# 0411tony/Yue

Hardware: AMD Instinct MI355X
Metric: BPR triplet-updates/sec at k=128 (S-round semantics, user rows sequential; the reference's exact sequential semantics: secondary.exact) (higher is better)
Workload: dtype f32

## Files before the change

include/yue_hip.h:

```cpp
#ifndef YUE_HIP_H
#define YUE_HIP_H

#include <stdint.h>

#ifdef __cplusplus
extern "C" {
#endif

typedef struct yue_ctx yue_ctx;

#define YUE_OK              0
#define YUE_ERR_ARG        -1
#define YUE_ERR_HIP        -2
#define YUE_ERR_FEW_ITEMS  -3
#define YUE_ERR_COMM       -4
#define YUE_ERR_SATURATED  -5

#define YUE_MAX_ATTEMPTS   64
#define YUE_UNIQUE_ID_BYTES 128

const char *yue_last_error(void);
int yue_version(void);

int yue_ctx_create(int device, yue_ctx **out);
// ... 19 lines not shown

int yue_bpr_rounds(yue_ctx *ctx, const int32_t *u, const int32_t *i, const int32_t *j,
                   const int64_t *round_ptr, int64_t n_rounds,
                   double lr, double regU, double regI, double *nll_out);

int yue_bpr_epoch(yue_ctx *ctx, uint64_t seed, uint32_t epoch, int64_t round_events,
                  double lr, double regU, double regI,
                  double *nll_out, double *sumsqP_out, double *sumsqQ_out);

int yue_epoch_plan(int64_t m, int k, int64_t round_events, double events_total, int nranks,
                   int64_t *user_block, int64_t *blocks_per_group, int64_t *n_blocks);

int yue_default_round_events(yue_ctx *ctx, int64_t *out);

int yue_sample_negatives(yue_ctx *ctx, uint64_t seed, uint32_t epoch, int32_t *j_out);

int yue_sumsq(yue_ctx *ctx, double *sumsqP_out, double *sumsqQ_out);

int yue_scores(yue_ctx *ctx, int32_t user, float *out_n);

int yue_topn_scan(yue_ctx *ctx, const int32_t *users, int64_t nu, int N,
                  const int64_t *mask_indptr, const int32_t *mask_indices,
                  int32_t *out_ids, float *out_scores);

int yue_set_kernel_timing(yue_ctx *ctx, int stride);
int yue_get_kernel_timing(yue_ctx *ctx, double *total_ms, int64_t *launches_timed, int64_t *triplets_timed);
int yue_get_scan_stats(yue_ctx *ctx, double *kernel_ms, int64_t *events, int64_t *rescored, int *used_bf16);
int yue_get_scan_work(yue_ctx *ctx, int64_t *tiles_scored, int64_t *tiles_total);

int yue_set_option(yue_ctx *ctx, const char *name, int64_t value);
// ... 99 lines not shown
```

yue_amd/_shim.py:

```python
import ctypes as C
import os

import numpy as np

_HERE = os.path.dirname(os.path.abspath(__file__))
LIB_PATH = os.path.join(_HERE, 'csrc', 'libyue_hip.so')

OK, ERR_ARG, ERR_HIP, ERR_FEW_ITEMS, ERR_COMM, ERR_SATURATED = 0, -1, -2, -3, -4, -5
UNIQUE_ID_BYTES = 128

SYMBOLS = ['yue_last_error', 'yue_version', 'yue_ctx_create', 'yue_ctx_destroy', 'yue_sync',
           'yue_set_factors', 'yue_get_factors', 'yue_set_interactions', 'yue_bpr_replay',
           'yue_bpr_rounds', 'yue_bpr_epoch', 'yue_cune_steps', 'yue_adam_reset', 'yue_adam_get_moments', 'yue_adam_step', 'yue_sample_negatives', 'yue_sumsq', 'yue_scores',
           'yue_topn_scan', 'yue_set_kernel_timing', 'yue_get_kernel_timing', 'yue_get_scan_stats', 'yue_get_scan_work', 'yue_set_option', 'yue_get_option',
           'yue_comm_unique_id', 'yue_comm_init', 'yue_allreduce_f64', 'yue_get_comm_stats',
           'yue_default_round_events', 'yue_epoch_plan',
           'yue_fism_set_model', 'yue_fism_get_model', 'yue_fism_epoch', 'yue_fism_rounds', 'yue_fism_scores', 'yue_fism_topn_scan',
           'yue_wrmf_set_pairs', 'yue_wrmf_half_sweep',
           'yue_expo_set_pairs', 'yue_expo_set_mu', 'yue_expo_get_mu', 'yue_expo_half_sweep', 'yue_expo_update_mu', 'yue_expo_gram_rows',
           'yue_cof_cooccur', 'yue_cof_get_cooccur', 'yue_cof_set_sppmi', 'yue_cof_set_state', 'yue_cof_get_state', 'yue_cof_item_sweep',
           'yue_knn_set_pairs', 'yue_knn_neighbors', 'yue_knn_predict', 'yue_knn_topn',
           'yue_ipf_set_graph', 'yue_ipf_predict', 'yue_ipf_topn',
           'yue_cnet_set_pairs', 'yue_cnet_walks', 'yue_cnet_set_walks', 'yue_cnet_set_sentences', 'yue_cnet_embed', 'yue_cnet_set_embedding',
           'yue_cnet_friends',
           'yue_s2v_set_state', 'yue_s2v_get_state', 'yue_s2v_set_steps', 'yue_s2v_set_pairs', 'yue_s2v_epoch',
           'yue_lgcn_set_graph', 'yue_lgcn_propagate', 'yue_lgcn_grad', 'yue_lgcn_step',
           'yue_ngcf_set_graph', 'yue_ngcf_set_weights', 'yue_ngcf_get_weights', 'yue_ngcf_propagate', 'yue_ngcf_grad', 'yue_ngcf_step',
           'yue_cdae_set_data', 'yue_cdae_set_params', 'yue_cdae_get_params', 'yue_cdae_forward', 'yue_cdae_grad', 'yue_cdae_step',
# ... 338 lines not shown
    def default_round_events(self):
        out = C.c_int64()
        self._chk(self._lib.yue_default_round_events(self._ctx, C.byref(out)))
        return out.value

    def bpr_epoch(self, seed, epoch, round_events, lr, regU, regI):
        nll, sp, sq = C.c_double(), C.c_double(), C.c_double()
        self._chk(self._lib.yue_bpr_epoch(self._ctx, C.c_uint64(seed), C.c_uint32(epoch), C.c_int64(round_events), C.c_double(lr), C.c_double(regU),
                                          C.c_double(regI), C.byref(nll), C.byref(sp), C.byref(sq)))
        return nll.value, sp.value, sq.value

    def sample_negatives(self, seed, epoch):
        j = np.empty(max(self.E, 1), np.int32)
        self._chk(self._lib.yue_sample_negatives(self._ctx, C.c_uint64(seed), C.c_uint32(epoch), j.ctypes.data_as(C.POINTER(C.c_int32))))
        return j[:self.E]

    def sumsq(self):
        sp, sq = C.c_double(), C.c_double()
        self._chk(self._lib.yue_sumsq(self._ctx, C.byref(sp), C.byref(sq)))
        return sp.value, sq.value

    def scores(self, user):
        out = np.empty(self.n, np.float32)
        self._chk(self._lib.yue_scores(self._ctx, C.c_int32(user), out.ctypes.data_as(C.POINTER(C.c_float))))
        return out

    def topn_scan(self, users, N, mask_indptr=None, mask_indices=None):
        users, up = _i32(users)
        ids = np.empty((len(users), N), np.int32)
        sc = np.empty((len(users), N), np.float32)
# ... 366 lines not shown
```

yue_amd/csrc/bpr_device.hpp:

```cpp
#pragma once
#include <hip/hip_runtime.h>
#include <stdint.h>

namespace yue {

constexpr int kNllSlots = 1024;
constexpr int kMaxAttempts = 64;

struct TrainArgs {
    float *P, *Q, *dP, *dQ;
    float *stage;
#ifdef YUE_STAMPS
    unsigned long long *stamps;
#endif
    const int32_t *ev_u, *ev_i;
    int32_t *ev_j;
    const int64_t *indptr;
    const int32_t *indices;
    double *nll_slots;
    int64_t m, n;
    int k;
    float ru, ri;
    double lr;
    uint64_t seed;
// ... 7 lines not shown
    unsigned long long *cnt_cur;
    unsigned long long *cnt_next;
    uint32_t *cntp_cur;
    uint32_t *cntp_next;
    uint32_t *tab_cur, *tab_next;
    int staged;
    int apply_p;
};

__device__ __forceinline__ uint64_t mix64(uint64_t z) {
    z ^= z >> 30; z *= 0xBF58476D1CE4E5B9ull;
    z ^= z >> 27; z *= 0x94D049BB133111EBull;
    z ^= z >> 31; return z;
}

__device__ __forceinline__ int32_t ctr_draw(uint64_t seed, uint32_t epoch, uint64_t e, uint32_t a, int32_t lo, int32_t n_range) {
    uint64_t z = mix64(seed + 0x9E3779B97F4A7C15ull * (e + 1));
    z = mix64(z ^ (0xD1B54A32D192ED03ull * (uint64_t)(epoch + 1) + 0x8CB92BA72F3D8DD7ull * (uint64_t)a));
    return lo + (int32_t)(((z >> 32) * (uint64_t)(uint32_t)n_range) >> 32);
}

__device__ __forceinline__ bool csr_contains(const int64_t *indptr, const int32_t *indices, int64_t row, int32_t x) {
    int64_t lo = indptr[row], hi = indptr[row + 1];
    while (lo < hi) {
        int64_t mid = (lo + hi) >> 1;
        int32_t v = indices[mid];
        if (v < x) lo = mid + 1; else if (v > x) hi = mid; else return true;
    }
    return false;
}

__device__ __forceinline__ int32_t sample_negative(const TrainArgs &a, int32_t u, int64_t e) {
    for (uint32_t t = 0; t < (uint32_t)kMaxAttempts; ++t) {
        int32_t c = ctr_draw(a.seed, a.epoch, (uint64_t)e, t, a.neg_lo, a.neg_range);
// ... 111 lines not shown
```

yue_amd/csrc/bpr_host.hip:

```cpp
#include "host_common.hpp"

#include "train_kernels.hpp"
#include "round_kernels.hpp"

using yue_host::fail;
using yue_host::kr_of;
using yue_host::with_kr;
static_assert(yue::kNllSlots == yue_host::kNllSlotsHost && yue::kHeaderSlack == yue_host::kHeaderSlackHost &&
              yue::kMetaStageMax == (uint32_t)yue_host::kMetaStageMaxHost, "host_common.hpp mirrors these");

namespace {

yue::TrainArgs make_args(yue_ctx *c, double lr, double regU, double regI) {
    yue::TrainArgs a{};
    a.P = c->P.p; a.Q = c->Q.p; a.dP = c->dP.p; a.dQ = c->dQ.p;
    a.stage = c->Q.p ? c->Q.p + (size_t)c->n * c->k : nullptr;
    a.ev_u = c->ev_u.p; a.ev_i = c->ev_i.p; a.ev_j = c->ev_j.p;
    a.indptr = c->indptr.p; a.indices = c->indices.p;
    a.nll_slots = c->scal.p;
    a.m = c->m; a.n = c->n; a.k = c->k;
    a.lr = lr;
    a.ru = (float)(lr * regU);
    a.ri = (float)(lr * regI);
    a.neg_lo = 0; a.neg_range = (int32_t)c->n;
// ... 182 lines not shown
            }
        });
        if (!is_default) return fail(YUE_ERR_ARG, "item matrices of 2 GiB and more: only the default events-per-wave setting (round_tpw = 0)");
    } else if (!with_round_instance(kr_of(c->k), tpw, [&](auto kr, auto t) {
                   hipLaunchKernelGGL((yue::k_round_m<kr(), t()>), grid, block, 0, c->stream, a, ra, a.ev_u, a.ev_i, a.ev_j, mi, mj);
               }))
        return fail(YUE_ERR_ARG, "unsupported (k, TPW) combination");
    launch_round_fold(c, a, e0, e1, round_index);
    return YUE_OK;
}

int launch_round_u(yue_ctx *c, const yue::TrainArgs &a, int64_t u0, int64_t u1, int64_t e0, int64_t e1, int64_t round_index) {
    yue::RoundUArgs ra{};
    ra.u_begin = u0; ra.u_end = u1; ra.ev_ptr = c->d_ev_ptr.p; ra.e_begin = e0; ra.e_end = e1; ra.staged = c->staged ? 1 : 0; ra.margins = c->margins.p;
    ra.psq_slots = c->psq_in_rounds ? c->psq_slots.p : nullptr;
    const int64_t blocks = (u1 - u0 + 3) / 4;
    if (blocks == 0) return YUE_OK;
    const dim3 grid((unsigned)blocks), block(256);
    const uint32_t *mi = c->meta_i.p, *mj = c->meta_j.p;
    with_kr(c->k, [&](auto kr) {
        if (c->opt_round_fast) hipLaunchKernelGGL((yue::k_round_u<kr(), true>), grid, block, 0, c->stream, a, ra, a.ev_i, a.ev_j, mi, mj);
        else hipLaunchKernelGGL((yue::k_round_u<kr(), false>), grid, block, 0, c->stream, a, ra, a.ev_i, a.ev_j, mi, mj);
    });
    launch_round_fold(c, a, e0, e1, round_index);
    return YUE_OK;
}

template <typename F>
int run_rounds(yue_ctx *c, yue::TrainArgs a, const std::vector<int64_t> &bounds, int apply_p, F after_round, bool meta = false, const std::vector<int64_t> *user_blocks = nullptr) {
    const int64_t R = (int64_t)bounds.size() - 1;
// ... 54 lines not shown
                      : meta ? launch_round_m(c, a, e0, e1, r) : launch_round(c, a, e0, e1, n0, n1, (int)(pos & 1), apply_p))) return rc;
            ++pos;
        }
        if ((rc = after_round(r))) return rc;
    }
    if (timed) {
        HIPCHK(hipEventRecord(c->ev_pool[c->ev_used].second, c->stream));
        c->ev_triplets[c->ev_used] = bounds.back() - bounds.front();
        c->ev_launches[c->ev_used] = (int64_t)ne.size();
        c->ev_used++;
    }
    return YUE_OK;
}

void reset_round_state(yue_ctx *c) {
    (void)hipStreamSynchronize(c->stream);
    if (c->cnt0.p) (void)hipMemsetAsync(c->cnt0.p, 0, c->cnt0.n * sizeof(unsigned long long), c->stream);
    if (c->cnt1.p) (void)hipMemsetAsync(c->cnt1.p, 0, c->cnt1.n * sizeof(unsigned long long), c->stream);
    if (c->cntp0.p) (void)hipMemsetAsync(c->cntp0.p, 0, c->cntp0.n * sizeof(uint32_t), c->stream);
    if (c->cntp1.p) (void)hipMemsetAsync(c->cntp1.p, 0, c->cntp1.n * sizeof(uint32_t), c->stream);
    if (c->dP.p) (void)hipMemsetAsync(c->dP.p, 0, c->dP.n * sizeof(float), c->stream);
    if (c->dQ.p) (void)hipMemsetAsync(c->dQ.p, 0, c->dQ.n * sizeof(float), c->stream);
    (void)hipStreamSynchronize(c->stream);
}

}

namespace yue_host {
bool fold_path(const yue_ctx *c) { return meta_path_fits(c); }

// ... 190 lines not shown
    int rc = upload_triplets(c, u, i, j, T, true);
    if (rc) return rc;
    if ((rc = zero_scalars(c))) return rc;
    yue::MbArgs a{};
    a.U = c->P.p; a.V = c->Q.p; a.gU = c->dP.p; a.gV = c->dQ.p; a.k = c->k; a.u = c->xu.p; a.i = c->xi.p; a.j = c->xj.p; a.T = T;
    a.reg = (float)reg; a.loss_slots = c->scal.p;
    const dim3 grid((unsigned)(((T + 31) / 32 + 3) / 4));
    with_kr(c->k, [&](auto kr) { hipLaunchKernelGGL(yue::k_mb_grad<kr()>, grid, dim3(256), 0, c->stream, a); });
    if ((rc = yue_host::adam_apply(c, lr, step))) return rc;
    return read_scalars(c, loss_out, nullptr, nullptr);
}

int yue_sample_negatives(yue_ctx *c, uint64_t seed, uint32_t epoch, int32_t *j_out) {
    if (!c || !c->have_inter || !j_out) return fail(YUE_ERR_ARG, "yue_sample_negatives: no interactions uploaded");
    HIPCHK(hipSetDevice(c->device));
    yue::TrainArgs a = make_args(c, 0, 0, 0);
    a.seed = seed; a.epoch = epoch;
    if (c->E > 0) {
        hipLaunchKernelGGL(yue::k_sample, dim3((unsigned)((c->E + 255) / 256)), dim3(256), 0, c->stream, a, c->E);
        HIPCHK(hipGetLastError());
        HIPCHK(hipMemcpyAsync(j_out, c->ev_j.p, c->E * sizeof(int32_t), hipMemcpyDeviceToHost, c->stream));
    }
    HIPCHK(hipStreamSynchronize(c->stream));
    return YUE_OK;
}

int yue_sumsq(yue_ctx *c, double *sp, double *sq) {
    if (!c || !c->have_factors) return fail(YUE_ERR_ARG, "yue_sumsq: no factors uploaded");
    HIPCHK(hipSetDevice(c->device));
    int rc = sumsq_async(c);
    if (rc) return rc;
    double h[2];
    HIPCHK(hipMemcpyAsync(h, c->scal.p + yue::kNllSlots + 1, sizeof h, hipMemcpyDeviceToHost, c->stream));
    HIPCHK(hipStreamSynchronize(c->stream));
    if (sp) *sp = h[0];
    if (sq) *sq = h[1];
    return YUE_OK;
}

int yue_bpr_epoch(yue_ctx *c, uint64_t seed, uint32_t epoch, int64_t round_events, double lr, double regU, double regI,
                  double *nll_out, double *sumsqP_out, double *sumsqQ_out) {
    if (!c || !c->have_factors || !c->have_inter) return fail(YUE_ERR_ARG, "yue_bpr_epoch: upload factors and interactions first");
    if (round_events < 0) return fail(YUE_ERR_ARG, "yue_bpr_epoch: round_events must be positive (or 0 for the device's default)");
    HIPCHK(hipSetDevice(c->device));
    yue::TrainArgs a = make_args(c, lr, regU, regI);
    a.seed = seed + 0x632BE59BD9B4E019ull * (uint64_t)c->rank;
    a.epoch = epoch;
    int rc = zero_scalars(c);
    if (rc) return rc;
    const int64_t E = c->E;
    if (E > 0) hipLaunchKernelGGL(yue::k_sample, dim3((unsigned)((E + 255) / 256)), dim3(256), 0, c->stream, a, E);
    if (c->opt_epoch_exact) {
        if (yue_host::on_communicator(c) && c->nranks > 1) return fail(YUE_ERR_ARG, "yue_bpr_epoch: option epoch_exact runs on one GPU (the sequential order spans all item shards)");
        if ((rc = yue_host::chain_epoch(c, lr, regU, regI))) return rc;
        if ((rc = sumsq_async(c))) return rc;
        return read_scalars(c, nll_out, sumsqP_out, sumsqQ_out);
    }
    std::vector<int64_t> bounds;
    double tot[2] = {(double)E, (double)c->n};
    if (yue_host::on_communicator(c)) {
        if ((rc = yue_allreduce_f64(c, tot, 2))) return rc;
        if ((rc = zero_scalars(c))) return rc;
    }
    const double etot = tot[0];
    if (round_events == 0 && (rc = default_round_events(c, tot[1] / c->nranks, &round_events))) return rc;
    int64_t ub = 1, group = 1;
// ... 26 lines not shown
        const int64_t first = g_first * c->k, count = (g_last - g_first) * c->k;
        const dim3 grid((unsigned)std::min<int64_t>(4096, (count + 255) / 256));
        if (!yue_host::on_communicator(c)) {
            hipLaunchKernelGGL(yue::k_apply_range, grid, dim3(256), 0, c->stream, c->P.p, c->dP.p, first, count);
            return YUE_OK;
        }
        HIPCHK(hipEventRecord(c->ev_rounds, c->stream));
        HIPCHK(hipStreamWaitEvent(c->comm_stream, c->ev_rounds, 0));
        c->comm_collectives += 1;
        c->comm_bytes += (double)count * sizeof(float);
        if (const int rcr = yue_host::reduce_user_block(c, first, count, c->comm_stream)) return rcr;
        hipLaunchKernelGGL(yue::k_apply_range, grid, dim3(256), 0, c->comm_stream, c->P.p, c->dP.p, first, count);
        return YUE_OK;
    };
    c->comm_collectives = 0; c->comm_bytes = 0.0; c->comm_wait_ms = 0.0;
    if ((rc = run_rounds(c, a, bounds, 0, after, meta_path_fits(c), seq_user ? &ublock : nullptr))) { reset_round_state(c); return rc; }
    if (c->last_round_user_seq && E > 0)
        hipLaunchKernelGGL(yue::k_loss_margins, dim3(2048), dim3(256), 0, c->stream, c->margins.p, c->ev_j.p, E, c->scal.p);
    const bool psq_done = c->psq_in_rounds && c->last_round_user_seq;
    c->psq_in_rounds = false;
    if (yue_host::on_communicator(c)) {
        HIPCHK(hipEventRecord(c->ev_t_rounds, c->stream));
        HIPCHK(hipEventRecord(c->ev_t_comm, c->comm_stream));
    }
    HIPCHK(hipEventRecord(c->ev_comm, c->comm_stream));
    HIPCHK(hipStreamWaitEvent(c->stream, c->ev_comm, 0));
    c->comm_compute_waits = 1;
    HIPCHK(hipGetLastError());
    if ((rc = sumsq_async(c, psq_done ? c->psq_slots.p : nullptr))) return rc;
    if ((rc = read_scalars(c, nll_out, sumsqP_out, sumsqQ_out))) return rc;
    if (yue_host::on_communicator(c)) {
        float ms = 0.f;
        HIPCHK(hipEventSynchronize(c->ev_t_comm));
        HIPCHK(hipEventElapsedTime(&ms, c->ev_t_rounds, c->ev_t_comm));
        c->comm_wait_ms = ms > 0.f ? ms : 0.0;
    }
    return YUE_OK;
}

int yue_epoch_plan(int64_t m, int k, int64_t round_events, double events_total, int nranks,
                   int64_t *user_block, int64_t *blocks_per_group, int64_t *n_blocks) {
    if (m <= 0 || k <= 0 || round_events <= 0 || nranks < 1 || !(events_total >= 0.0)) return fail(YUE_ERR_ARG, "yue_epoch_plan: bad argument");
    const double per_user = events_total / (double)nranks / (double)m;
    const int64_t ub = std::max<int64_t>(1, (int64_t)std::floor((double)round_events / std::max(per_user, 1e-9) + 0.5));
    if (user_block) *user_block = ub;
    if (blocks_per_group) *blocks_per_group = std::max<int64_t>(1, (8ll << 20) / std::max<int64_t>(1, ub * k * 4));
    if (n_blocks) *n_blocks = (m + ub - 1) / ub;
    return YUE_OK;
}

int yue_default_round_events(yue_ctx *c, int64_t *out) {
// ... 50 lines not shown
```

yue_amd/csrc/core_host.hip:

```cpp
#include "host_common.hpp"

namespace yue_host {
thread_local std::string g_err;
int fail(int code, const std::string &msg) { g_err = msg; return code; }
}
using yue_host::fail;
void yue_comm_release(yue_ctx *c);

extern "C" {

const char *yue_last_error(void) { return yue_host::g_err.c_str(); }
int yue_version(void) { return 1; }

int yue_ctx_create(int device, yue_ctx **out) {
    if (!out) return fail(YUE_ERR_ARG, "yue_ctx_create: out is NULL");
    int ndev = 0;
    HIPCHK(hipGetDeviceCount(&ndev));
    if (ndev <= 0) return fail(YUE_ERR_HIP, "no HIP device visible: libyue_hip needs an MI355X (no CPU fallback exists)");
    if (device < 0 || device >= ndev) return fail(YUE_ERR_ARG, "device ordinal out of range");
    HIPCHK(hipSetDevice(device));
    yue_ctx *c = new yue_ctx();
    c->device = device;
    const auto init = [c]() -> int {
        HIPCHK(hipStreamCreateWithFlags(&c->stream, hipStreamNonBlocking));
// ... 21 lines not shown
    yue_comm_release(c);
    if (c->comm_stream) (void)hipStreamDestroy(c->comm_stream);
    if (c->ev_rounds) (void)hipEventDestroy(c->ev_rounds);
    if (c->ev_comm) (void)hipEventDestroy(c->ev_comm);
    if (c->ev_t_rounds) (void)hipEventDestroy(c->ev_t_rounds);
    if (c->ev_t_comm) (void)hipEventDestroy(c->ev_t_comm);
    if (c->ev_scan0) (void)hipEventDestroy(c->ev_scan0);
    if (c->ev_chain0) (void)hipEventDestroy(c->ev_chain0);
    if (c->ev_chain1) (void)hipEventDestroy(c->ev_chain1);
    if (c->ev_scan1) (void)hipEventDestroy(c->ev_scan1);
    for (auto &pr : c->ev_pool) { (void)hipEventDestroy(pr.first); (void)hipEventDestroy(pr.second); }
    c->P.release(); c->Q.release(); c->dP.release(); c->dQ.release(); c->margins.release();
    c->cnt0.release(); c->cnt1.release(); c->cntp0.release(); c->cntp1.release();
    c->tab0.release(); c->tab1.release();
    c->meta_i.release(); c->meta_j.release(); c->round_rows.release(); c->d_bounds.release(); c->fold.release(); c->bk_touch.release(); c->bk_ptr.release();
    c->ev_u.release(); c->ev_i.release(); c->ev_j.release(); c->indices.release(); c->indptr.release();
    c->xu.release(); c->xi.release(); c->xj.release(); c->xk.release(); c->x_loss.release(); c->scal.release();
    c->aU_m.release(); c->aU_v.release(); c->aV_m.release(); c->aV_v.release();
    c->s_users.release(); c->s_ids.release(); c->s_mask_idx.release(); c->s_flags.release();
    c->s_mask_ptr.release(); c->s_scores.release(); c->s_row.release(); c->s_norms.release(); c->s_work.release(); c->s_qb.release(); c->s_masks.release(); c->s_few.release(); c->s_few_ids.release(); c->s_few_scores.release();
    c->fP.release(); c->fBi.release(); c->f_coef.release(); c->f_x.release(); c->f_hist.release(); c->f_scores.release();
    c->f_out_sc.release(); c->fQ.release(); c->f_ptr.release(); c->f_items.release(); c->f_negs.release(); c->f_ids.release(); c->f_flags.release();
    c->f_uq_ptr.release(); c->f_neg_ptr.release(); c->f_uq_items.release(); c->f_loc_i.release(); c->f_loc_j.release();
    c->f_wq.release(); c->f_dQ.release(); c->f_wp.release(); c->f_wb.release(); c->f_dP.release(); c->f_dB.release();
    c->ch_key.release(); c->ch_val.release(); c->ch_key2.release(); c->ch_val2.release(); c->ch_seg.release(); c->ch_ord_i.release(); c->ch_ord_j.release();
    c->ch_head.release(); c->ch_incl.release(); c->ch_ord_u.release(); c->ch_rkey.release(); c->ch_rval.release(); c->ch_run_ptr.release(); c->d_ev_ptr.release();
    c->ch_run_u.release(); c->ch_tmp.release(); c->ch_Qv.release(); c->ch_Pv.release(); c->ch_ctl.release(); c->ch_stats.release();
    yue_host::wrmf_release(c);
    yue_host::knn_release(c);
    yue_host::ipf_release(c);
    yue_host::expo_release(c);
// ... 62 lines not shown
        }
        if (indptr[u + 1] - indptr[u] >= n) return fail(YUE_ERR_ARG, "yue_set_interactions: a user listened to every item (the reference's sampler would never return, BPR.py:47)");
    }
    const int64_t nnz = indptr[m], E = ev_ptr[m];
    {
        int64_t prev = -1, max_gap = 0;
        for (int64_t u = 0; u < m; ++u) if (ev_ptr[u + 1] > ev_ptr[u]) { if (prev >= 0) max_gap = std::max(max_gap, u - prev); prev = u; }
        if (max_gap * c->k * 4 >= (1ll << 31)) return fail(YUE_ERR_ARG, "yue_set_interactions: more than 2 GiB of user-factor rows between two consecutive users with events");
    }
    std::vector<int32_t> evu((size_t)E);
    for (int64_t u = 0; u < m; ++u)
        for (int64_t e = ev_ptr[u]; e < ev_ptr[u + 1]; ++e) {
            if (ev_i[e] < 0 || ev_i[e] >= n) return fail(YUE_ERR_ARG, "yue_set_interactions: event item out of range");
            evu[(size_t)e] = (int32_t)u;
        }
    c->E = E; c->nnz = nnz;
    c->h_ev_ptr.assign(ev_ptr, ev_ptr + m + 1);
    c->all_users_have_events = true;
    for (int64_t u = 0; u < m; ++u) if (ev_ptr[u + 1] <= ev_ptr[u]) { c->all_users_have_events = false; break; }
    c->d_ev_ptr_valid = false;
    HIPCHK(c->indptr.resize(m + 1)); HIPCHK(c->indices.resize(std::max<int64_t>(nnz, 1)));
    HIPCHK(c->ev_u.resize((size_t)E + yue_host::kHeaderSlackHost)); HIPCHK(c->ev_i.resize((size_t)E + yue_host::kHeaderSlackHost)); HIPCHK(c->ev_j.resize((size_t)E + yue_host::kHeaderSlackHost));
    HIPCHK(hipMemcpyAsync(c->indptr.p, indptr, (m + 1) * sizeof(int64_t), hipMemcpyHostToDevice, c->stream));
    HIPCHK(hipMemcpyAsync(c->indices.p, indices, nnz * sizeof(int32_t), hipMemcpyHostToDevice, c->stream));
    HIPCHK(hipMemcpyAsync(c->ev_u.p, evu.data(), E * sizeof(int32_t), hipMemcpyHostToDevice, c->stream));
    HIPCHK(hipMemcpyAsync(c->ev_i.p, ev_i, E * sizeof(int32_t), hipMemcpyHostToDevice, c->stream));
    HIPCHK(hipStreamSynchronize(c->stream));
    c->have_inter = true;
    return YUE_OK;
}
// ... 4 lines not shown
```

yue_amd/csrc/host_common.hpp:

```cpp
#pragma once
#include "../../include/yue_hip.h"

#include <hip/hip_runtime.h>

#include <algorithm>
#include <cmath>
#include <cstdio>
#include <cstdlib>
#include <cstring>
#include <string>
#include <type_traits>
#include <vector>

struct ncclComm;
struct yue_wrmf;
struct yue_knn;
struct yue_expo;
struct yue_cof;
struct yue_cnet;
struct yue_s2v;
struct yue_lgcn;
struct yue_ngcf;
struct yue_cdae;
struct yue_ipf;
// ... 57 lines not shown
    DevBuf<uint32_t> tab0, tab1;
    bool staged = false;
    bool bigq = false;
    DevBuf<uint32_t> meta_i, meta_j;
    DevBuf<unsigned long long> round_rows;
    DevBuf<uint2> fold, bk_touch;
    DevBuf<uint32_t> bk_ptr;
    DevBuf<int64_t> d_bounds;
    std::vector<int64_t> h_bounds;
#ifdef YUE_STAMPS
    DevBuf<unsigned long long> stamps;
    int64_t stamp_launch = -1, update_launches = 0, stamp_waves = 0;
#endif
    DevBuf<int32_t> ev_u, ev_i, ev_j, indices;
    DevBuf<int64_t> indptr;
    DevBuf<int32_t> xu, xi, xj, xk;
    DevBuf<double> x_loss;
    DevBuf<float> aU_m, aU_v, aV_m, aV_v;
    int64_t adam_m = 0, adam_n = 0; int adam_k = 0;
    DevBuf<double> scal;
    std::vector<int64_t> h_ev_ptr;
    bool all_users_have_events = false;
    bool psq_in_rounds = false;
    DevBuf<int32_t> s_users, s_ids, s_mask_idx, s_flags;
    DevBuf<int32_t> s_few, s_few_ids;
    DevBuf<float> s_few_scores;
    int64_t scan_few_users = 0;
    DevBuf<int64_t> s_mask_ptr;
    DevBuf<float> s_scores, s_row, s_norms;
    double scan_ms = 0.0;
// ... 143 lines not shown
```

yue_amd/csrc/options_host.hip:

```cpp
#include "host_common.hpp"

#include <limits>

using yue_host::fail;

namespace {

struct Option {
    const char *name;
    int64_t (*get)(yue_ctx *);
    void (*put)(yue_ctx *, int64_t);
    int (*set)(const Option &, yue_ctx *, int64_t);
    int64_t lo, hi;
    const char *refusal;
    std::vector<int64_t> also;
};
#define YUE_AT(member) [](yue_ctx *c) -> int64_t { return c->member; }, [](yue_ctx *c, int64_t v) { c->member = (decltype(c->member))v; }

int set_flag(const Option &o, yue_ctx *c, int64_t value) { o.put(c, value != 0); return YUE_OK; }

int set_ranged(const Option &o, yue_ctx *c, int64_t value) {
    if ((value < o.lo || value > o.hi) && std::find(o.also.begin(), o.also.end(), value) == o.also.end())
        return fail(YUE_ERR_ARG, std::string("yue_set_option: ") + o.name + " " + o.refusal);
    o.put(c, value);
// ... 45 lines not shown
    {"scan_last_chunks", YUE_AT(scan_chunks)},
    {"scan_last_few_users", YUE_AT(scan_few_users)},
    {"scan_last_settle", YUE_AT(scan_settle)},
    {"topn_true", YUE_AT(opt_topn_true), set_flag},
    {"fism_lds", YUE_AT(opt_fism_lds), set_flag},
    {"fism_inplace", YUE_AT(opt_fism_inplace), set_flag},
    {"round_stage", YUE_AT(opt_round_stage), set_ranged, 0, yue_host::kMetaStageMaxHost, "must be 0, 1 or 2..64"},
    {"round_last_stage_max", YUE_AT(last_stage_max)},
    {"round_meta", YUE_AT(opt_round_meta), set_flag},
    {"comm_group_mb", YUE_AT(opt_comm_group_mb), set_ranged, 1, 4096, "must be 1..4096"},
    {"round_cus_reserved", YUE_AT(opt_round_cus_reserved), set_round_cus_reserved},
    {"comm_last_compute_waits", YUE_AT(comm_compute_waits)},
    {"round_user_seq", YUE_AT(opt_round_user_seq), set_flag},
    {"round_fast", YUE_AT(opt_round_fast), set_flag},
    {"round_last_user_seq", YUE_AT(last_round_user_seq)},
    {"round_bucket", YUE_AT(opt_round_bucket), set_flag},
    {"fold_blocks", YUE_AT(opt_fold_blocks), set_ranged, 1, 65536, "out of range"},
    {"round_tpw", YUE_AT(opt_round_tpw), set_round_tpw},
    {"round_path", round_path},
#ifdef YUE_STAMPS
    {"debug_stamp_launch", nullptr, nullptr, set_stamp_launch},
#endif
    {"epoch_exact", YUE_AT(opt_epoch_exact), set_flag},
    {"replay_levels", YUE_AT(opt_replay_levels), set_flag},
    {"chain_waves", YUE_AT(opt_chain_waves), set_ranged, 0, 8, "must be 0..8"},
    {"chain_split", YUE_AT(opt_chain_split), set_ranged, -1, 1, "must be -1, 0 or 1"},
    {"chain_fast", YUE_AT(opt_chain_fast), set_flag},
    {"chain_xcd", YUE_AT(opt_chain_xcd), set_flag},
    {"chain_ring", YUE_AT(opt_chain_ring), set_ranged, 0, 0, "must be 0, 8 or 16", {8, 16}},
    {"chain_spin", YUE_AT(opt_chain_spin), set_ranged, 0, 0x7fffffff, "out of range"},
// ... 68 lines not shown
```

yue_amd/csrc/round_kernels.hpp:

```cpp
#pragma once
#include "train_kernels.hpp"

#ifdef YUE_ABL_NO_HOT
#define YUE_M_HOT(val, rs, vo, so) asm volatile("" :: "v"(val))
#else
#define YUE_M_HOT(val, rs, vo, so) YUE_BATOMIC(val, rs, vo, so)
#endif
#ifdef YUE_ABL_NO_DP
#define YUE_M_DP(val, rs, vo, so) asm volatile("" :: "v"(val))
#else
#define YUE_M_DP(val, rs, vo, so) YUE_BATOMIC(val, rs, vo, so)
#endif

#define YUE_BLOAD_NT(rs, vo, so) __builtin_bit_cast(float, __builtin_amdgcn_raw_buffer_load_b32((rs), (vo), (so), 2))
#if defined(YUE_EXP_LOAD_CACHED)
#define YUE_M_LOAD_J(rs, vo, so) YUE_BLOAD(rs, vo, so)
#define YUE_M_LOAD_I(rs, vo, so) YUE_BLOAD(rs, vo, so)
#elif defined(YUE_EXP_LOAD_NT)
#define YUE_M_LOAD_J(rs, vo, so) YUE_BLOAD_NT(rs, vo, so)
#define YUE_M_LOAD_I(rs, vo, so) YUE_BLOAD_NT(rs, vo, so)
#else
#define YUE_M_LOAD_J(rs, vo, so) YUE_BLOAD_NT(rs, vo, so)
#define YUE_M_LOAD_I(rs, vo, so) YUE_BLOAD(rs, vo, so)
#endif
// ... 378 lines not shown
    }
    YUE_STAMP(4, ""); YUE_STAMP(5, ""); YUE_STAMP(6, "");
#pragma unroll
    for (int off = 1; off < TPW; off <<= 1) nll += __shfl_xor(nll, off);
    if (lane == 0 && nll != 0.0) atomicAdd(a.nll_slots + (wave & (kNllSlots - 1)), nll);
    YUE_STAMP(7, "s_waitcnt vmcnt(0)");
}

struct RoundUArgs {
    int64_t u_begin, u_end;
    const int64_t *ev_ptr;
    int64_t e_begin, e_end;
    int staged;
    float *margins;
    double *psq_slots;
};

template <int KR, bool FAST>
__global__ void __launch_bounds__(256) k_round_u(TrainArgs a, RoundUArgs ra, const int32_t *__restrict__ evi, const int32_t *__restrict__ evj,
                                                 const uint32_t *__restrict__ mti, const uint32_t *__restrict__ mtj) {
    const int lane = threadIdx.x & 63;
    const int64_t wave = (int64_t)blockIdx.x * 4 + __builtin_amdgcn_readfirstlane((int)(threadIdx.x >> 6));
    const int64_t u = ra.u_begin + wave;
    if (u >= ra.u_end) return;
    const int64_t e0 = ra.ev_ptr[u], e1 = ra.ev_ptr[u + 1];
    if (e1 <= e0) return;
    const unsigned k = (unsigned)a.k;
    const unsigned row_bytes = k * 4u;
    unsigned vo[KR];
#pragma unroll
    for (int r = 0; r < KR; ++r) { const unsigned e = 64u * r + lane; vo[r] = e < k ? e * 4u : kOobOffset; }
    const uint64_t qbytes = (uint64_t)a.n * row_bytes;
    const int qrec = (int)(qbytes < 0x7fffffffull ? qbytes : 0x7fffffffull);
    const unsigned stage0 = (unsigned)a.n * row_bytes;
    const uint64_t qsbytes = qbytes + (ra.staged ? 2ull * (uint64_t)(ra.e_end - ra.e_begin) * row_bytes : 0ull);
    const int qsrec = (int)(qsbytes < 0x7fffffffull ? qsbytes : 0x7fffffffull);
    const auto rsQ = __builtin_amdgcn_make_buffer_rsrc(a.Q, 0, qsrec, kRsrcFlags);
    const auto rsdQ = __builtin_amdgcn_make_buffer_rsrc(a.dQ, 0, qrec, kRsrcFlags);
    float *prow = a.P + (uint64_t)u * k;
    float p[KR];
#pragma unroll
    for (int r = 0; r < KR; ++r) { const unsigned e = 64u * r + lane; p[r] = e < k ? prow[e] : 0.0f; }
    const float lrf = (float)a.lr;
    const unsigned len = (unsigned)(e1 - e0 < 0x7fffffff ? e1 - e0 : 0x7fffffff);
    for (unsigned seg = 0; seg < len; seg += 64u) {
        int hI, hJ;
        uint32_t hMI, hMJ;
        {
            const bool ex = seg + (unsigned)lane < len;
            const int64_t e = e0 + seg + (ex ? lane : 0);
            hI = evi[e]; hJ = evj[e]; hMI = mti[e]; hMJ = mtj[e];
            if (!ex) { hI = 0; hJ = -1; hMI = 0u; hMJ = 0u; }
        }
        const unsigned seg_len = len - seg < 64u ? len - seg : 64u;
        float xs = 0.0f;
        auto gather = [&](float (&qi)[KR], float (&qj)[KR], unsigned t) {
            const int ti = __builtin_amdgcn_readlane(hI, t), tj = __builtin_amdgcn_readlane(hJ, t);
            const unsigned oi = (unsigned)ti * row_bytes, oj = (unsigned)(tj < 0 ? 0 : tj) * row_bytes;
#pragma unroll
// ... 26 lines not shown
#pragma unroll
                for (int r = 0; r < KR; ++r) YUE_M_HOT(o[r].qi2 - qi[r], rsdQ, vo[r], oi);
            }
            if (clj != kMetaHot) {
#pragma unroll
                for (int r = 0; r < KR; ++r) YUE_BSTORE(full_j ? o[r].qj2 : o[r].qj2 - qj[r], rsQ, vo[r], wj);
            } else {
#pragma unroll
                for (int r = 0; r < KR; ++r) YUE_M_HOT(o[r].qj2 - qj[r], rsdQ, vo[r], oj);
            }
        };
        constexpr int D = KR == 1 ? 8 : 4;
        float qi[D][KR], qj[D][KR];
#pragma unroll
        for (int s_ = 0; s_ < D; ++s_) gather(qi[s_], qj[s_], (unsigned)s_);
        for (unsigned t = 0; t < seg_len; t += D) {
#pragma unroll
            for (int s_ = 0; s_ < D; ++s_) {
                step(qi[s_], qj[s_], t + s_);
                gather(qi[s_], qj[s_], (t + s_ + D) & 63u);
            }
        }
        if ((unsigned)lane < seg_len) ra.margins[e0 + seg + lane] = xs;
    }
#pragma unroll
    for (int r = 0; r < KR; ++r) { const unsigned e = 64u * r + lane; if (e < k) prow[e] = p[r]; }
    if (ra.psq_slots) {
        double s = 0.0;
#pragma unroll
        for (int r = 0; r < KR; ++r) { const unsigned e = 64u * r + lane; const float sq = p[r] * p[r]; if (e < k) s += (double)sq; }
#pragma unroll
        for (int off = 1; off < 64; off <<= 1) s += __shfl_xor(s, off);
        if (lane == 0) atomicAdd(ra.psq_slots + (u & (kNllSlots - 1)), s);
    }
}

__global__ void __launch_bounds__(256) k_loss_margins(const float *__restrict__ x, const int32_t *__restrict__ evj, int64_t E, double *nll_slots) {
    double nl = 0.0;
    const int64_t stride = (int64_t)gridDim.x * blockDim.x;
    for (int64_t e = (int64_t)blockIdx.x * blockDim.x + threadIdx.x; e < E; e += stride)
        if (evj[e] >= 0) nl += -log(chain_sigmoid(x[e]));
#pragma unroll
    for (int off = 1; off < 64; off <<= 1) nl += __shfl_xor(nl, off);
    if ((threadIdx.x & 63) == 0 && nl != 0.0) atomicAdd(nll_slots + ((blockIdx.x * 4 + (threadIdx.x >> 6)) & (kNllSlots - 1)), nl);
}

struct FoldArgs {
    const uint2 *fold;
// ... 121 lines not shown
```

Before: 1.841 billion.

## Draw next epoch's negatives inside the user-sequential round kernel

During the user-sequential round kernel, each wave also samples the next epoch's negative items for its events. It checks candidates against the user's positives, using register readlane compares when the user fits in one segment and a CSR search otherwise, and writes them to a second buffer. The next bpr_epoch call then swaps buffers and skips the separate k_sample launch, which the host verifies by seed, epoch, range and interaction generation. This removes a standalone sampling pass over all events in exchange for extra ALU work and register pressure in the round kernel, plus an SGPR cap attribute.

```diff
diff --git a/include/yue_hip.h b/include/yue_hip.h
--- a/include/yue_hip.h
+++ b/include/yue_hip.h
@@ -57,6 +57,8 @@
 int yue_default_round_events(yue_ctx *ctx, int64_t *out);
 
 int yue_sample_negatives(yue_ctx *ctx, uint64_t seed, uint32_t epoch, int32_t *j_out);
+
+int yue_bpr_prefetched_negatives(yue_ctx *ctx, uint64_t *seed, uint32_t *epoch, int32_t *j_out);
 
 int yue_sumsq(yue_ctx *ctx, double *sumsqP_out, double *sumsqQ_out);
 
diff --git a/yue_amd/_shim.py b/yue_amd/_shim.py
--- a/yue_amd/_shim.py
+++ b/yue_amd/_shim.py
@@ -11,7 +11,7 @@
 
 SYMBOLS = ['yue_last_error', 'yue_version', 'yue_ctx_create', 'yue_ctx_destroy', 'yue_sync',
            'yue_set_factors', 'yue_get_factors', 'yue_set_interactions', 'yue_bpr_replay',
-           'yue_bpr_rounds', 'yue_bpr_epoch', 'yue_cune_steps', 'yue_adam_reset', 'yue_adam_get_moments', 'yue_adam_step', 'yue_sample_negatives', 'yue_sumsq', 'yue_scores',
+           'yue_bpr_rounds', 'yue_bpr_epoch', 'yue_cune_steps', 'yue_adam_reset', 'yue_adam_get_moments', 'yue_adam_step', 'yue_sample_negatives', 'yue_bpr_prefetched_negatives', 'yue_sumsq', 'yue_scores',
            'yue_topn_scan', 'yue_set_kernel_timing', 'yue_get_kernel_timing', 'yue_get_scan_stats', 'yue_get_scan_work', 'yue_set_option', 'yue_get_option',
            'yue_comm_unique_id', 'yue_comm_init', 'yue_allreduce_f64', 'yue_get_comm_stats',
            'yue_default_round_events', 'yue_epoch_plan',
@@ -380,6 +380,12 @@
         j = np.empty(max(self.E, 1), np.int32)
         self._chk(self._lib.yue_sample_negatives(self._ctx, C.c_uint64(seed), C.c_uint32(epoch), j.ctypes.data_as(C.POINTER(C.c_int32))))
         return j[:self.E]
+
+    def prefetched_negatives(self):
+        seed, epoch = C.c_uint64(), C.c_uint32()
+        j = np.empty(max(self.E, 1), np.int32)
+        self._chk(self._lib.yue_bpr_prefetched_negatives(self._ctx, C.byref(seed), C.byref(epoch), j.ctypes.data_as(C.POINTER(C.c_int32))))
+        return seed.value, epoch.value, j[:self.E]
 
     def sumsq(self):
         sp, sq = C.c_double(), C.c_double()
diff --git a/yue_amd/csrc/bpr_device.hpp b/yue_amd/csrc/bpr_device.hpp
--- a/yue_amd/csrc/bpr_device.hpp
+++ b/yue_amd/csrc/bpr_device.hpp
@@ -45,10 +45,13 @@
     z ^= z >> 31; return z;
 }
 
+__device__ __forceinline__ uint64_t ctr_event(uint64_t seed, uint64_t e) { return mix64(seed + 0x9E3779B97F4A7C15ull * (e + 1)); }
+__device__ __forceinline__ int32_t ctr_attempt(uint64_t ze, uint32_t epoch, uint32_t a, int32_t lo, int32_t n_range) {
+    const uint64_t z = mix64(ze ^ (0xD1B54A32D192ED03ull * (uint64_t)(epoch + 1) + 0x8CB92BA72F3D8DD7ull * (uint64_t)a));
+    return lo + (int32_t)(((z >> 32) * (uint64_t)(uint32_t)n_range) >> 32);
+}
 __device__ __forceinline__ int32_t ctr_draw(uint64_t seed, uint32_t epoch, uint64_t e, uint32_t a, int32_t lo, int32_t n_range) {
-    uint64_t z = mix64(seed + 0x9E3779B97F4A7C15ull * (e + 1));
-    z = mix64(z ^ (0xD1B54A32D192ED03ull * (uint64_t)(epoch + 1) + 0x8CB92BA72F3D8DD7ull * (uint64_t)a));
-    return lo + (int32_t)(((z >> 32) * (uint64_t)(uint32_t)n_range) >> 32);
+    return ctr_attempt(ctr_event(seed, e), epoch, a, lo, n_range);
 }
 
 __device__ __forceinline__ bool csr_contains(const int64_t *indptr, const int32_t *indices, int64_t row, int32_t x) {
diff --git a/yue_amd/csrc/bpr_host.hip b/yue_amd/csrc/bpr_host.hip
--- a/yue_amd/csrc/bpr_host.hip
+++ b/yue_amd/csrc/bpr_host.hip
@@ -220,6 +220,7 @@
     yue::RoundUArgs ra{};
     ra.u_begin = u0; ra.u_end = u1; ra.ev_ptr = c->d_ev_ptr.p; ra.e_begin = e0; ra.e_end = e1; ra.staged = c->staged ? 1 : 0; ra.margins = c->margins.p;
     ra.psq_slots = c->psq_in_rounds ? c->psq_slots.p : nullptr;
+    ra.next_j = c->next_j_out; ra.next_epoch = c->next_j_epoch;
     const int64_t blocks = (u1 - u0 + 3) / 4;
     if (blocks == 0) return YUE_OK;
     const dim3 grid((unsigned)blocks), block(256);
@@ -304,6 +305,7 @@
 }
 
 void reset_round_state(yue_ctx *c) {
+    c->prefetch.valid = false;
     (void)hipStreamSynchronize(c->stream);
     if (c->cnt0.p) (void)hipMemsetAsync(c->cnt0.p, 0, c->cnt0.n * sizeof(unsigned long long), c->stream);
     if (c->cnt1.p) (void)hipMemsetAsync(c->cnt1.p, 0, c->cnt1.n * sizeof(unsigned long long), c->stream);
@@ -524,6 +526,7 @@
 int yue_sample_negatives(yue_ctx *c, uint64_t seed, uint32_t epoch, int32_t *j_out) {
     if (!c || !c->have_inter || !j_out) return fail(YUE_ERR_ARG, "yue_sample_negatives: no interactions uploaded");
     HIPCHK(hipSetDevice(c->device));
+    c->prefetch.valid = false;
     yue::TrainArgs a = make_args(c, 0, 0, 0);
     a.seed = seed; a.epoch = epoch;
     if (c->E > 0) {
@@ -531,6 +534,17 @@
         HIPCHK(hipGetLastError());
         HIPCHK(hipMemcpyAsync(j_out, c->ev_j.p, c->E * sizeof(int32_t), hipMemcpyDeviceToHost, c->stream));
     }
+    HIPCHK(hipStreamSynchronize(c->stream));
+    return YUE_OK;
+}
+
+int yue_bpr_prefetched_negatives(yue_ctx *c, uint64_t *seed, uint32_t *epoch, int32_t *j_out) {
+    if (!c || !c->have_inter || !seed || !epoch || !j_out) return fail(YUE_ERR_ARG, "yue_bpr_prefetched_negatives: null argument or no interactions uploaded");
+    if (!c->prefetch.valid || c->prefetch.generation != c->inter_generation)
+        return fail(YUE_ERR_ARG, "yue_bpr_prefetched_negatives: no epoch's negatives are held in advance");
+    HIPCHK(hipSetDevice(c->device));
+    *seed = c->prefetch.seed; *epoch = c->prefetch.epoch;
+    if (c->E > 0) HIPCHK(hipMemcpyAsync(j_out, c->ev_j_next.p, c->E * sizeof(int32_t), hipMemcpyDeviceToHost, c->stream));
     HIPCHK(hipStreamSynchronize(c->stream));
     return YUE_OK;
 }
@@ -559,7 +573,18 @@
     int rc = zero_scalars(c);
     if (rc) return rc;
     const int64_t E = c->E;
-    if (E > 0) hipLaunchKernelGGL(yue::k_sample, dim3((unsigned)((E + 255) / 256)), dim3(256), 0, c->stream, a, E);
+    const bool u_path = !c->opt_epoch_exact && !yue_host::on_communicator(c) && c->opt_round_user_seq && meta_path_fits(c);
+    const bool prefetch = u_path && c->opt_round_prefetch_neg && c->ev_items_are_rows && E > 0;
+    const bool prefetched = prefetch && c->prefetch.valid && c->prefetch.seed == a.seed && c->prefetch.epoch == epoch &&
+                            c->prefetch.neg_lo == a.neg_lo && c->prefetch.neg_range == a.neg_range && c->prefetch.generation == c->inter_generation;
+    c->prefetch.valid = false;
+    c->last_round_prefetched = prefetched ? 1 : 0;
+    if (prefetched) {
+        std::swap(c->ev_j, c->ev_j_next);
+        a.ev_j = c->ev_j.p;
+    } else if (E > 0) {
+        hipLaunchKernelGGL(yue::k_sample, dim3((unsigned)((E + 255) / 256)), dim3(256), 0, c->stream, a, E);
+    }
     if (c->opt_epoch_exact) {
         if (yue_host::on_communicator(c) && c->nranks > 1) return fail(YUE_ERR_ARG, "yue_bpr_epoch: option epoch_exact runs on one GPU (the sequential order spans all item shards)");
         if ((rc = yue_host::chain_epoch(c, lr, regU, regI))) return rc;
@@ -616,7 +641,14 @@
         return YUE_OK;
     };
     c->comm_collectives = 0; c->comm_bytes = 0.0; c->comm_wait_ms = 0.0;
-    if ((rc = run_rounds(c, a, bounds, 0, after, meta_path_fits(c), seq_user ? &ublock : nullptr))) { reset_round_state(c); return rc; }
+    if (prefetch) {
+        HIPCHK(c->ev_j_next.resize((size_t)E + yue::kHeaderSlack));
+        c->next_j_out = c->ev_j_next.p; c->next_j_epoch = epoch + 1;
+    }
+    rc = run_rounds(c, a, bounds, 0, after, meta_path_fits(c), seq_user ? &ublock : nullptr);
+    const bool drew_next = c->next_j_out && c->last_round_user_seq;
+    c->next_j_out = nullptr;
+    if (rc) { reset_round_state(c); return rc; }
     if (c->last_round_user_seq && E > 0)
         hipLaunchKernelGGL(yue::k_loss_margins, dim3(2048), dim3(256), 0, c->stream, c->margins.p, c->ev_j.p, E, c->scal.p);
     const bool psq_done = c->psq_in_rounds && c->last_round_user_seq;
@@ -637,6 +669,11 @@
         HIPCHK(hipEventElapsedTime(&ms, c->ev_t_rounds, c->ev_t_comm));
         c->comm_wait_ms = ms > 0.f ? ms : 0.0;
     }
+    if (drew_next) {
+        c->prefetch.seed = a.seed; c->prefetch.epoch = epoch + 1; c->prefetch.neg_lo = a.neg_lo; c->prefetch.neg_range = a.neg_range;
+        c->prefetch.generation = c->inter_generation;
+        c->prefetch.valid = true;
+    }
     return YUE_OK;
 }
 
diff --git a/yue_amd/csrc/core_host.hip b/yue_amd/csrc/core_host.hip
--- a/yue_amd/csrc/core_host.hip
+++ b/yue_amd/csrc/core_host.hip
@@ -59,7 +59,7 @@
     c->cnt0.release(); c->cnt1.release(); c->cntp0.release(); c->cntp1.release();
     c->tab0.release(); c->tab1.release();
     c->meta_i.release(); c->meta_j.release(); c->round_rows.release(); c->d_bounds.release(); c->fold.release(); c->bk_touch.release(); c->bk_ptr.release();
-    c->ev_u.release(); c->ev_i.release(); c->ev_j.release(); c->indices.release(); c->indptr.release();
+    c->ev_u.release(); c->ev_i.release(); c->ev_j.release(); c->ev_j_next.release(); c->indices.release(); c->indptr.release();
     c->xu.release(); c->xi.release(); c->xj.release(); c->xk.release(); c->x_loss.release(); c->scal.release();
     c->aU_m.release(); c->aU_v.release(); c->aV_m.release(); c->aV_v.release();
     c->s_users.release(); c->s_ids.release(); c->s_mask_idx.release(); c->s_flags.release();
@@ -152,6 +152,22 @@
             if (ev_i[e] < 0 || ev_i[e] >= n) return fail(YUE_ERR_ARG, "yue_set_interactions: event item out of range");
             evu[(size_t)e] = (int32_t)u;
         }
+    c->prefetch.valid = false;
+    c->prefetch.generation = ++c->inter_generation;
+    c->ev_items_are_rows = true;
+    {
+        std::vector<int64_t> mark((size_t)n, -1);
+        for (int64_t u = 0; u < m && c->ev_items_are_rows; ++u) {
+            for (int64_t t = indptr[u]; t < indptr[u + 1]; ++t) mark[(size_t)indices[t]] = 2 * u;
+            int64_t distinct = 0;
+            for (int64_t e = ev_ptr[u]; e < ev_ptr[u + 1]; ++e) {
+                int64_t &w = mark[(size_t)ev_i[e]];
+                if (w == 2 * u) { w = 2 * u + 1; ++distinct; }
+                else if (w != 2 * u + 1) c->ev_items_are_rows = false;
+            }
+            if (distinct != indptr[u + 1] - indptr[u]) c->ev_items_are_rows = false;
+        }
+    }
     c->E = E; c->nnz = nnz;
     c->h_ev_ptr.assign(ev_ptr, ev_ptr + m + 1);
     c->all_users_have_events = true;
diff --git a/yue_amd/csrc/host_common.hpp b/yue_amd/csrc/host_common.hpp
--- a/yue_amd/csrc/host_common.hpp
+++ b/yue_amd/csrc/host_common.hpp
@@ -95,6 +95,20 @@
 #endif
     DevBuf<int32_t> ev_u, ev_i, ev_j, indices;
     DevBuf<int64_t> indptr;
+    DevBuf<int32_t> ev_j_next;
+    struct {
+        bool valid = false;
+        uint64_t seed = 0;
+        uint32_t epoch = 0;
+        int32_t neg_lo = 0, neg_range = 0;
+        int64_t generation = 0;
+    } prefetch;
+    int64_t inter_generation = 0;
+    bool ev_items_are_rows = false;
+    int32_t *next_j_out = nullptr;
+    uint32_t next_j_epoch = 0;
+    int opt_round_prefetch_neg = 1;
+    int last_round_prefetched = 0;
     DevBuf<int32_t> xu, xi, xj, xk;
     DevBuf<double> x_loss;
     DevBuf<float> aU_m, aU_v, aV_m, aV_v;
diff --git a/yue_amd/csrc/options_host.hip b/yue_amd/csrc/options_host.hip
--- a/yue_amd/csrc/options_host.hip
+++ b/yue_amd/csrc/options_host.hip
@@ -83,6 +83,8 @@
     {"round_user_seq", YUE_AT(opt_round_user_seq), set_flag},
     {"round_fast", YUE_AT(opt_round_fast), set_flag},
     {"round_last_user_seq", YUE_AT(last_round_user_seq)},
+    {"round_prefetch_neg", YUE_AT(opt_round_prefetch_neg), set_flag},
+    {"round_last_prefetched", YUE_AT(last_round_prefetched)},
     {"round_bucket", YUE_AT(opt_round_bucket), set_flag},
     {"fold_blocks", YUE_AT(opt_fold_blocks), set_ranged, 1, 65536, "out of range"},
     {"round_tpw", YUE_AT(opt_round_tpw), set_round_tpw},
diff --git a/yue_amd/csrc/round_kernels.hpp b/yue_amd/csrc/round_kernels.hpp
--- a/yue_amd/csrc/round_kernels.hpp
+++ b/yue_amd/csrc/round_kernels.hpp
@@ -416,10 +416,39 @@
     int staged;
     float *margins;
     double *psq_slots;
+    int32_t *next_j;
+    uint32_t next_epoch;
 };
 
+__device__ __forceinline__ int32_t draw_next_negative(const TrainArgs &a, uint32_t next_epoch, int64_t u, int64_t e, bool mine,
+                                                      bool one_segment, int hI, unsigned seg_len) {
+    const uint64_t ze = ctr_event(a.seed, (uint64_t)e);
+    const int items = mine ? hI : -1;
+    int32_t jn = -1;
+    bool open = mine;
+    for (uint32_t at = 0; at < (uint32_t)kMaxAttempts && __builtin_amdgcn_ballot_w64(open) != 0ull; ++at) {
+        const int32_t cand = ctr_attempt(ze, next_epoch, at, a.neg_lo, a.neg_range);
+        bool hit = false;
+        if (one_segment) {
+            unsigned miss = 0xffffffffu;
+#pragma unroll
+            for (unsigned g = 0; g < 64u; g += 8u) {
+                if (g < seg_len) {
+#pragma unroll
+                    for (unsigned t = g; t < g + 8u; ++t) miss = min(miss, (unsigned)(cand ^ __builtin_amdgcn_readlane(items, t)));
+                }
+            }
+            hit = miss == 0u;
+        } else if (open) {
+            hit = csr_contains(a.indptr, a.indices, u, cand);
+        }
+        if (open && !hit) { jn = cand; open = false; }
+    }
+    return jn;
+}
+
 template <int KR, bool FAST>
-__global__ void __launch_bounds__(256) k_round_u(TrainArgs a, RoundUArgs ra, const int32_t *__restrict__ evi, const int32_t *__restrict__ evj,
+__global__ void __launch_bounds__(256) __attribute__((amdgpu_num_sgpr(80))) k_round_u(TrainArgs a, RoundUArgs ra, const int32_t *__restrict__ evi, const int32_t *__restrict__ evj,
                                                  const uint32_t *__restrict__ mti, const uint32_t *__restrict__ mtj) {
     const int lane = threadIdx.x & 63;
     const int64_t wave = (int64_t)blockIdx.x * 4 + __builtin_amdgcn_readfirstlane((int)(threadIdx.x >> 6));
@@ -445,6 +474,13 @@
     for (int r = 0; r < KR; ++r) { const unsigned e = 64u * r + lane; p[r] = e < k ? prow[e] : 0.0f; }
     const float lrf = (float)a.lr;
     const unsigned len = (unsigned)(e1 - e0 < 0x7fffffff ? e1 - e0 : 0x7fffffff);
+    auto draw_next = [&](unsigned seg, unsigned seg_len, int hI) {
+        if (!ra.next_j) return;
+        const bool mine = (unsigned)lane < seg_len;
+        const int64_t e = e0 + seg + lane;
+        const int32_t jn = draw_next_negative(a, ra.next_epoch, u, e, mine, len <= 64u, hI, seg_len);
+        if (mine) ra.next_j[e] = jn;
+    };
     for (unsigned seg = 0; seg < len; seg += 64u) {
         int hI, hJ;
         uint32_t hMI, hMJ;
@@ -501,6 +537,7 @@
         float qi[D][KR], qj[D][KR];
 #pragma unroll
         for (int s_ = 0; s_ < D; ++s_) gather(qi[s_], qj[s_], (unsigned)s_);
+        if (KR < 4) draw_next(seg, seg_len, hI);
         for (unsigned t = 0; t < seg_len; t += D) {
 #pragma unroll
             for (int s_ = 0; s_ < D; ++s_) {
@@ -519,6 +556,13 @@
 #pragma unroll
         for (int off = 1; off < 64; off <<= 1) s += __shfl_xor(s, off);
         if (lane == 0) atomicAdd(ra.psq_slots + (u & (kNllSlots - 1)), s);
+    }
+    if (KR == 4 && ra.next_j) {
+        for (unsigned seg = 0; seg < len; seg += 64u) {
+            const unsigned seg_len = len - seg < 64u ? len - seg : 64u;
+            const int hI = (unsigned)lane < seg_len ? evi[e0 + seg + lane] : 0;
+            draw_next(seg, seg_len, hI);
+        }
     }
 }
 
```

After: 1.892 billion, median of 6. 1.03x the previous value.
